# ap229997/hands

Hardware: AMD Instinct MI355X
Metric: hands/sec (higher is better)
Workload: dtype f32; 1 GPU; hands_light ResNet-50 x3 + feature_conv + HMR + MANO, 224x224, bz=256 samples/GPU (512 hands, 768 trunk passes); per_gpu_batch=256, global_batch=256, parallelism=dp1, rccl_ranks=1, launched_by=direct, conv3x3_stride1=winograd_f4x4:stages1234

## Files before the change

### hands_amd/csrc/common.h

```cpp
#pragma once
#include <hip/hip_runtime.h>
#include <math.h>

#define HANDS_LAUNCH_CHECK() return (int)hipGetLastError()

static inline int hands_grid_1d(long long work, int block, int cap = 256 * 8) {
  long long g = (work + block - 1) / block;
  if (g < 1) g = 1;
  if (g > cap) g = cap;
  return (int)g;
}

typedef float f32x4 __attribute__((ext_vector_type(4)));
typedef float f32x16 __attribute__((ext_vector_type(16)));

__device__ __forceinline__ float f4e(const float4& v, int t) {
  return t == 0 ? v.x : (t == 1 ? v.y : (t == 2 ? v.z : v.w));
}

__device__ __forceinline__ float relu_f32(float v) { return v <= 0.f ? 0.f : v; }
__device__ __forceinline__ float4 relu_f32(const float4& v) {
  return make_float4(relu_f32(v.x), relu_f32(v.y), relu_f32(v.z), relu_f32(v.w));
}
struct PoolNan4 { bool x = false, y = false, z = false, w = false; };
__device__ __forceinline__ void pool_tap(float4& m, PoolNan4& seen, const float4& v) {
  m.x = fmaxf(m.x, v.x); m.y = fmaxf(m.y, v.y); m.z = fmaxf(m.z, v.z); m.w = fmaxf(m.w, v.w);
  seen.x |= v.x != v.x; seen.y |= v.y != v.y; seen.z |= v.z != v.z; seen.w |= v.w != v.w;
}
__device__ __forceinline__ float4 pool_finish(const float4& m, const PoolNan4& seen) {
  const float q = __builtin_nanf("");
  return make_float4(seen.x ? q : m.x, seen.y ? q : m.y, seen.z ? q : m.z, seen.w ? q : m.w);
}

__device__ __forceinline__ float exp_nonpos(float x) {
  const float L2E_HI = 1.44269502162933349609375f, L2E_LO = 1.925963033500011e-08f;
// ... 61 lines not shown
```

### hands_amd/csrc/conv_igemm.hip

```cpp
#include <hip/hip_runtime.h>
#include <stdint.h>
#include "hands_hip.h"
#include "common.h"

namespace {

typedef unsigned int u32x4 __attribute__((ext_vector_type(4)));
typedef double f64x4 __attribute__((ext_vector_type(4)));

__device__ __forceinline__ float gelu_erf(float x) { return x * 0.5f * (1.0f + erff(x * 0.70710678118654752440f)); }

__device__ __forceinline__ float4 apply_act(float4 v, int act) {
  if (act == HANDS_ACT_RELU) {
    v = relu_f32(v);
  } else if (act == HANDS_ACT_GELU) {
    v.x = gelu_erf(v.x); v.y = gelu_erf(v.y); v.z = gelu_erf(v.z); v.w = gelu_erf(v.w);
  } else if (act == HANDS_ACT_LEAKY_RELU) {
    v.x = v.x > 0.f ? v.x : 0.01f * v.x; v.y = v.y > 0.f ? v.y : 0.01f * v.y;
    v.z = v.z > 0.f ? v.z : 0.01f * v.z; v.w = v.w > 0.f ? v.w : 0.01f * v.w;
  }
  return v;
}

__device__ __forceinline__ float f4elem(const float4& v, int t) {
// ... 13 lines not shown
  const float r2 = r1 - __uint_as_float(u1);
  u2 = __float_as_uint(r2);
}

__device__ __forceinline__ void store_split4(float* dst, float4 v) {
  uint32_t a0, a1, a2, b0, b1, b2, c0, c1, c2, d0, d1, d2;
  split3(v.x, a0, a1, a2); split3(v.y, b0, b1, b2); split3(v.z, c0, c1, c2); split3(v.w, d0, d1, d2);
  *reinterpret_cast<uint2*>(dst) = make_uint2((a0 >> 16) | b0, (c0 >> 16) | d0);
  *reinterpret_cast<uint2*>(dst + 8) = make_uint2((a1 >> 16) | b1, (c1 >> 16) | d1);
  *reinterpret_cast<uint2*>(dst + 16) = make_uint2((a2 >> 16) | (b2 & 0xffff0000u), (c2 >> 16) | (d2 & 0xffff0000u));
}

struct ConvArgs {
  const float* __restrict__ in;
  const float* __restrict__ w;
  const float* __restrict__ bias;
  const float* res;
  float* out;
  int M, N, Kpad;
  int H, W, Cin, Ho, Wo, KH, KW, stride, pad;
  int in_ps, out_ps, res_ps;
  int relu;
  int nblk_m, nblk_n;
  const float* __restrict__ in2;
  int K0, H2, W2, stride2, in2_ps;
  int ksplit;
  float* partial;
  int part_ps;
  const float* pre_scale;
  const float* pre_shift;
  int* counters = nullptr;
  const float* fin_res = nullptr;
  int fin_act = 0;
};

__device__ __forceinline__ int xcd_remap(int bid, int nwg) {
  const int q = nwg >> 3, r = nwg & 7;
  const int xcd = bid & 7, idx = bid >> 3;
  const int base = (xcd < r) ? xcd * (q + 1) : r * (q + 1) + (xcd - r) * q;
  return base + idx;
}

typedef float f32x2 __attribute__((ext_vector_type(2)));

constexpr int EROW = 68;
constexpr int EPI_FLOATS = 4 * 32 * EROW;
template <int ACT, bool RES>
__device__ __forceinline__ void epilogue_full(const f32x16 (&acc)[2][2], float* sE, int lane, const float* bias_p,
                                              const char* res_u, int res_ps, char* out_u, int out_ps) {
  const int half = lane >> 5;
  float* wr = sE + (lane & 31) * EROW + half * 4;
  const float* rd = sE + (lane >> 4) * EROW + (lane & 15) * 4;
  const uint32_t o_off = (uint32_t)((lane >> 4) * out_ps + (lane & 15) * 4) * 4u;
  const uint32_t r_off = (uint32_t)((lane >> 4) * res_ps + (lane & 15) * 4) * 4u;
  const float4 bv4 = *reinterpret_cast<const float4*>(bias_p);
#ifndef HANDS_EPI_SCALAR_ADDS
  const f32x2 b01 = {bv4.x, bv4.y}, b23 = {bv4.z, bv4.w};
#endif
#pragma unroll
  for (int j = 0; j < 2; ++j) {
#pragma unroll
    for (int i = 0; i < 2; ++i)
#pragma unroll
      for (int q = 0; q < 4; ++q)
        *reinterpret_cast<float4*>(wr + i * 32 + q * 8) =
            make_float4(acc[i][j][q * 4 + 0], acc[i][j][q * 4 + 1], acc[i][j][q * 4 + 2], acc[i][j][q * 4 + 3]);
    float4 rv[RES ? 8 : 1];
// ... 56 lines not shown
      float f = (float)(v + (double)a.bias[n]);
      if (a.fin_res) f += a.fin_res[(size_t)m * a.res_ps + n];
      if (a.fin_act == HANDS_ACT_RELU) f = relu_f32(f);
      else if (a.fin_act == HANDS_ACT_GELU) f = gelu_erf(f);
      else if (a.fin_act == HANDS_ACT_LEAKY_RELU) f = f > 0.f ? f : 0.01f * f;
      a.out[(size_t)m * a.out_ps + n] = f;
    }
  } else {
    constexpr int C4 = BN / 4;
    for (int idx = tid; idx < BM * C4; idx += 256) {
      const int m = m0 + idx / C4, n = n0 + (idx % C4) * 4;
      if (m >= a.M || n >= a.N) continue;
      const float* p = a.partial + (size_t)m * a.part_ps + n;
      float4 v = *reinterpret_cast<const float4*>(p);
      for (int sl = 1; sl < a.ksplit; ++sl) {
        const float4 q = *reinterpret_cast<const float4*>(p + sl * slice);
        v.x += q.x; v.y += q.y; v.z += q.z; v.w += q.w;
      }
      const float4 b = *reinterpret_cast<const float4*>(a.bias + n);
      v.x += b.x; v.y += b.y; v.z += b.z; v.w += b.w;
      if (a.fin_res) {
        const float4 r = *reinterpret_cast<const float4*>(a.fin_res + (size_t)m * a.res_ps + n);
        v.x += r.x; v.y += r.y; v.z += r.z; v.w += r.w;
      }
      *reinterpret_cast<float4*>(a.out + (size_t)m * a.out_ps + n) = apply_act(v, a.fin_act);
    }
  }
}

constexpr int SK_SLOT_FLOATS = 4 * 64 * 64;

__device__ __forceinline__ void tile_coords(const ConvArgs& a, int tile, int& mt, int& nt) {
  constexpr int RASTER_GM = 8;
  if (a.nblk_n >= 8 && a.nblk_m >= RASTER_GM) {
    const int per = RASTER_GM * a.nblk_n;
    const int gidx = tile / per, idx = tile - gidx * per;
    const int gm = min(RASTER_GM, a.nblk_m - gidx * RASTER_GM);
    nt = idx / gm; mt = gidx * RASTER_GM + (idx - nt * gm);
  } else { mt = tile / a.nblk_n; nt = tile - mt * a.nblk_n; }
}

template <int WAVES_M, int WAVES_N, int MODE, int PREC = 0, bool PRE = false, int BLK = 0>
__device__ __forceinline__ void conv_tile(const ConvArgs& a, float* lds, int tile, int split, int kt0, int kt1,
                                          const float* acc_in, float* acc_out) {
  constexpr int ROW = PREC == 1 ? LDS_ROW_B3 : LDS_ROW;
  constexpr bool F64 = PREC == 2;
  constexpr bool STEM = MODE == 1;
  constexpr bool DUAL = MODE == 2;
  constexpr int BM = 64 * WAVES_M;
  constexpr int BN = 64 * WAVES_N;
  constexpr int A_ROWS = BM / 64;
  constexpr int W_ROWS = BN / 64;
  static_assert(WAVES_M * WAVES_N == 4, "4 waves per block");

  float* sX = lds;
  float* sW = lds + 2 * BM * ROW;

  const int tid = threadIdx.x;
  const int lane = tid & 63;
  const int wave = tid >> 6;
  const int wm = wave / WAVES_N;
  const int wn = wave % WAVES_N;

  int mt, nt;
  tile_coords(a, tile, mt, nt);
  const int m0 = mt * BM, n0 = nt * BN;

  const int srow = tid >> 2;
  const int chunk = tid & 3;
  const int swz_chunk = chunk ^ ((srow >> 2) & 3);
  int x_base[A_ROWS];
  int x_hi0[A_ROWS], x_wi0[A_ROWS];
  bool x_ok[A_ROWS];
  int x_base2[DUAL ? A_ROWS : 1];
  uint32_t x_mask[MODE == 0 ? A_ROWS : 1];
  int x_offb[MODE == 0 ? A_ROWS : 1];
  int x_b[A_ROWS];
  const int HoWo = a.Ho * a.Wo;
  const bool same_pixel = DUAL && a.K0 >= a.Kpad && a.stride == 1 && a.H == a.Ho && a.W == a.Wo;
#pragma unroll
  for (int i = 0; i < A_ROWS; ++i) {
    const int m = m0 + srow + 64 * i;
    x_ok[i] = m < a.M;
    const int mm = x_ok[i] ? m : 0;
    if (same_pixel) {
      x_b[i] = 0; x_hi0[i] = 0; x_wi0[i] = 0;
      x_base[i] = mm * a.in_ps;
      if constexpr (DUAL) x_base2[i] = 0;
      continue;
    }
    const int b = mm / HoWo;
    const int rem = mm - b * HoWo;
    const int ho = rem / a.Wo;
    const int wo = rem - ho * a.Wo;
    x_b[i] = b;
    x_hi0[i] = ho * a.stride - a.pad;
    x_wi0[i] = wo * a.stride - a.pad;
    x_base[i] = ((b * a.H + x_hi0[i]) * a.W + x_wi0[i]) * a.in_ps;
    if constexpr (DUAL) {
      x_base2[i] = ((b * a.H2 + ho * a.stride2) * a.W2 + wo * a.stride2) * a.in2_ps;
    }
  }
  __amdgpu_buffer_rsrc_t x_rsrc = __builtin_amdgcn_make_buffer_rsrc(const_cast<float*>(a.in), 0, (int)0x80000000u, 0x00020000);
  if constexpr (MODE == 0) {
    const int b_w = __builtin_amdgcn_readfirstlane(x_b[0]);
    x_rsrc = __builtin_amdgcn_make_buffer_rsrc(const_cast<float*>(a.in) + (size_t)b_w * a.H * a.W * a.in_ps, 0,
                                               (int)0x80000000u, 0x00020000);
#pragma unroll
    for (int i = 0; i < A_ROWS; ++i) {
      const int hb = max(0, -x_hi0[i]), he = min(a.KH, a.H - x_hi0[i]);
      const int wb = max(0, -x_wi0[i]), we = min(a.KW, a.W - x_wi0[i]);
      const uint32_t hm = he > hb ? ((1u << he) - 1u) & ~((1u << hb) - 1u) : 0u;
      const uint32_t wm = we > wb ? ((1u << we) - 1u) & ~((1u << wb) - 1u) : 0u;
      x_mask[i] = (x_ok[i] && hm != 0u && wm != 0u) ? (hm | (wm << 16)) : 0u;
      x_offb[i] = (((((x_b[i] - b_w) * a.H + x_hi0[i]) * a.W + x_wi0[i]) * a.in_ps) + chunk * 4) * 4;
    }
  }
  int x_off1[DUAL ? A_ROWS : 1], x_off2[DUAL ? A_ROWS : 1];
  __amdgpu_buffer_rsrc_t x_rsrc2 = x_rsrc;
  if constexpr (DUAL) {
    const int base1 = __builtin_amdgcn_readfirstlane(x_base[0]);
    const int base2 = __builtin_amdgcn_readfirstlane(x_base2[0]);
    x_rsrc = __builtin_amdgcn_make_buffer_rsrc(const_cast<float*>(a.in) + base1, 0, (int)0x80000000u, 0x00020000);
    x_rsrc2 = __builtin_amdgcn_make_buffer_rsrc(const_cast<float*>(a.in2) + base2, 0, (int)0x80000000u, 0x00020000);
#pragma unroll
    for (int i = 0; i < A_ROWS; ++i) {
      x_off1[i] = x_ok[i] ? (x_base[i] - base1 + chunk * 4) * 4 : chunk * 16;
      x_off2[i] = x_ok[i] ? (x_base2[i] - base2 + chunk * 4) * 4 : chunk * 16;
    }
  }
  const __amdgpu_buffer_rsrc_t w_rsrc =
      __builtin_amdgcn_make_buffer_rsrc(const_cast<float*>(a.w) + (size_t)n0 * a.Kpad, 0, (int)0x80000000u, 0x00020000);
  int w_offb[W_ROWS];
#pragma unroll
  for (int i = 0; i < W_ROWS; ++i) w_offb[i] = ((srow + 64 * i) * a.Kpad + chunk * 4) * 4;

  float4 xr[A_ROWS], wr[W_ROWS];
  static_assert(!PRE || (MODE == 2 && PREC != 1), "the input affine + LeakyReLU exists for exact-fp32 pointwise layers");
  float4 psr = make_float4(1.f, 1.f, 1.f, 1.f), pbr = make_float4(0.f, 0.f, 0.f, 0.f);
  int kh = 0, kw = 0, c0 = 0, woff = 0;
  const int ntaps = a.KH * a.KW;
  const int cw = (a.Cin & 31) == 0 ? 2 * BK : BK;

#define LOAD_TILES(KT)                                                                              \
  do {                                                                                              \
    if constexpr (STEM) {                                                                           \
                                          \
      const int tap = (KT) * 4 + chunk;                                                             \
      const int tkh = tap / a.KW;                                                                   \
      const int tkw = tap - tkh * a.KW;                                                             \
      const int toff = (tkh * a.W + tkw) * a.in_ps;                                                 \
      _Pragma("unroll") for (int i = 0; i < A_ROWS; ++i) {                                          \
        const bool ok = x_ok[i] && tap < ntaps && (unsigned)(x_hi0[i] + tkh) < (unsigned)a.H &&     \
                        (unsigned)(x_wi0[i] + tkw) < (unsigned)a.W;                                 \
        xr[i] = ok ? *reinterpret_cast<const float4*>(a.in + (x_base[i] + toff))                    \
                   : make_float4(0.f, 0.f, 0.f, 0.f);                                               \
      }                                                                                             \
    } else if constexpr (DUAL) {                                                                    \
       \
       \
       \
      const bool second = (KT) * BK >= a.K0;                                                        \
      const int soff = ((KT) * BK - (second ? a.K0 : 0)) * 4;                                       \
      _Pragma("unroll") for (int i = 0; i < A_ROWS; ++i) {                                          \
        const u32x4 ld = second ? __builtin_amdgcn_raw_buffer_load_b128(x_rsrc2, x_off2[i], soff, 0) \
                                : __builtin_amdgcn_raw_buffer_load_b128(x_rsrc, x_off1[i], soff, 0);  \
        xr[i] = make_float4(__uint_as_float(ld.x), __uint_as_float(ld.y), __uint_as_float(ld.z), __uint_as_float(ld.w)); \
      }                                                                                             \
    } else {                                                                                        \
       \
       \
       \
      const bool kvalid = c0 < a.Cin;              \
      const uint32_t sel = kvalid ? ((1u << kh) | (0x10000u << kw)) : 0x80000000u;   \
      const int toffb = ((kh * a.W + kw) * a.in_ps + c0) * 4;                                       \
      _Pragma("unroll") for (int i = 0; i < A_ROWS; ++i) {                                          \
        const bool ok = (x_mask[i] & sel) == sel;                                                   \
        const u32x4 ld = __builtin_amdgcn_raw_buffer_load_b128(x_rsrc, ok ? x_offb[i] + toffb : (int)0x80000000u, 0, 0); \
        xr[i] = make_float4(__uint_as_float(ld.x), __uint_as_float(ld.y), __uint_as_float(ld.z), __uint_as_float(ld.w)); \
      }                                                                                             \
      woff = kvalid ? (kh * a.KW + kw) * a.Cin + c0 : (KT) * BK;                                    \
      c0 += BK;                                                                                     \
      if ((c0 & (cw - 1)) == 0) {              \
        c0 -= cw;                                                                                   \
        if (++kw == a.KW) { kw = 0; if (++kh == a.KH) { kh = 0; c0 += cw; } }                       \
      }                                                                                             \
    }                                                                                               \
    if constexpr (MODE != 0) woff = (KT) * BK;                                                      \
    if constexpr (PRE) {                                                                            \
// ... 279 lines not shown
#pragma unroll
    for (int i = 0; i < 2; ++i)
#pragma unroll
      for (int q = 0; q < 4; ++q)
        *reinterpret_cast<float4*>(sE + (lane & 31) * EROW + i * 32 + q * 8 + half * 4) =
            make_float4(acc[i][j][q * 4 + 0], acc[i][j][q * 4 + 1], acc[i][j][q * 4 + 2], acc[i][j][q * 4 + 3]);
    }
    const int mbase = m0 + wm * 64 + j * 32 + (lane >> 4);
    float4 rv[8];
#pragma unroll
    for (int r = 0; r < 8; ++r) {
      const int m = mbase + 4 * r;
      const int mc = m < a.M ? m : a.M - 1;
      rv[r] = has_res ? *reinterpret_cast<const float4*>(a.res + (size_t)mc * a.res_ps + (n_ok ? n_lane : 0))
                      : make_float4(0.f, 0.f, 0.f, 0.f);
    }
#pragma unroll
    for (int r = 0; r < 8; ++r) {
      const int m = mbase + 4 * r;
      const float4 t = *reinterpret_cast<const float4*>(sE + ((lane >> 4) + 4 * r) * EROW + c4 * 4);
      float4 v;
      v.x = t.x + bv.x + rv[r].x;
      v.y = t.y + bv.y + rv[r].y;
      v.z = t.z + bv.z + rv[r].z;
      v.w = t.w + bv.w + rv[r].w;
      v = apply_act(v, act);
      if (m < a.M && n_ok) *reinterpret_cast<float4*>(obase + (size_t)m * ops + n_lane) = v;
    }
  }
#undef LOAD_TILES
#undef STORE_TILES
}

template <int WAVES_M, int WAVES_N, int MODE, int PREC = 0, bool PRE = false, int BLK = 0>
__global__ void __launch_bounds__(256, 2) conv_igemm_f32_kernel(ConvArgs a) {
  constexpr int RING = 2 * (64 * WAVES_M + 64 * WAVES_N) * (PREC == 1 ? LDS_ROW_B3 : LDS_ROW);
  __shared__ __attribute__((aligned(16))) float lds[RING > EPI_FLOATS ? RING : EPI_FLOATS];
  const int ntiles = a.nblk_m * a.nblk_n;
  const int split = a.ksplit > 1 ? blockIdx.x / ntiles : 0;
  const int tile = xcd_remap(a.ksplit > 1 ? blockIdx.x - split * ntiles : blockIdx.x, ntiles);
  const int nk_all = a.Kpad / BK;
  const int kt0 = a.ksplit > 1 ? (int)((long long)split * nk_all / a.ksplit) : 0;
  const int kt1 = a.ksplit > 1 ? (int)((long long)(split + 1) * nk_all / a.ksplit) : nk_all;
  const int wave_u = __builtin_amdgcn_readfirstlane((int)(threadIdx.x >> 6));
  conv_tile<WAVES_M, WAVES_N, MODE, PREC, PRE, BLK>(a, lds, tile, split, kt0, kt1, nullptr, nullptr);
  if (a.ksplit > 1 && a.counters != nullptr) {
    int mt, nt;
    tile_coords(a, tile, mt, nt);
    splitk_fused_tail<64 * WAVES_M, 64 * WAVES_N, PREC == 2>(a, lds, tile, mt * 64 * WAVES_M, nt * 64 * WAVES_N, wave_u);
  }
}

constexpr int GROUP_MAX = 8;
struct GroupArgs {
  ConvArgs a[GROUP_MAX];
  int start[GROUP_MAX + 1];
  int n;
};

template <int WAVES_M, int WAVES_N, int MODE, bool PRE, int BLK>
__global__ void __launch_bounds__(256, 2) conv_igemm_group_f32_kernel(GroupArgs g) {
  constexpr int RING = 2 * (64 * WAVES_M + 64 * WAVES_N) * LDS_ROW;
  __shared__ __attribute__((aligned(16))) float lds[RING > EPI_FLOATS ? RING : EPI_FLOATS];
  int p = 0;
#pragma unroll
  for (int i = 1; i < GROUP_MAX; ++i)
    if (i < g.n && (int)blockIdx.x >= g.start[i]) p = i;
  const ConvArgs& a = g.a[p];
  const int ntiles = a.nblk_m * a.nblk_n;
  const int local = (int)blockIdx.x - g.start[p];
  if ((local >> 3) >= (ntiles >> 3) + ((local & 7) < (ntiles & 7) ? 1 : 0)) return;
  conv_tile<WAVES_M, WAVES_N, MODE, 0, PRE, BLK>(a, lds, xcd_remap(local, ntiles), 0, 0, a.Kpad / BK, nullptr, nullptr);
}

struct SkArgs {
  float* slots;
  int* flags;
  int epoch;
};

template <int WAVES_M, int WAVES_N, int MODE>
__global__ void __launch_bounds__(256, 2) conv_igemm_sk_f32_kernel(ConvArgs a, SkArgs sk) {
  constexpr int RING = 2 * (64 * WAVES_M + 64 * WAVES_N) * LDS_ROW;
  __shared__ __attribute__((aligned(16))) float lds[RING > EPI_FLOATS ? RING : EPI_FLOATS];
  __shared__ int s_ready;
  const int G = gridDim.x;
  const int g = xcd_remap(blockIdx.x, G);
  const int ntiles = a.nblk_m * a.nblk_n;
  const int nk = a.Kpad / BK;
  const long long total = (long long)ntiles * nk;
  const long long u0 = total * g / G, u1 = total * (g + 1) / G;
// ... 16 lines not shown
      tile = first_full + (sgi - head);
    } else if (inside && ka == 0) {
      tile = ta; k1 = kb;
      aout = sk.slots + (size_t)g * SK_SLOT_FLOATS;
    } else {
      if (threadIdx.x == 0) {
        int ok = 0;
        for (int spin = 0; spin < 4096 && !ok; ++spin) {
          ok = __hip_atomic_load(sk.flags + (g - 1), __ATOMIC_RELAXED, __HIP_MEMORY_SCOPE_AGENT) == sk.epoch;
          if (!ok) __builtin_amdgcn_s_sleep(8);
        }
        if (ok) __builtin_amdgcn_fence(__ATOMIC_ACQUIRE, "agent");
        s_ready = ok;
      }
      __syncthreads();
      tile = ta;
      if (s_ready != 0) { k0 = ka; ain = sk.slots + (size_t)(g - 1) * SK_SLOT_FLOATS; }
      if (inside) { k1 = kb; aout = sk.slots + (size_t)g * SK_SLOT_FLOATS; }
    }
    __syncthreads();
    conv_tile<WAVES_M, WAVES_N, MODE>(a, lds, tile, 0, k0, k1, ain, aout);
    if (aout != nullptr) {
      asm volatile("s_waitcnt vmcnt(0)" ::: "memory");
      __syncthreads();
      if (threadIdx.x == 0) {
        __builtin_amdgcn_fence(__ATOMIC_RELEASE, "agent");
        asm volatile("s_waitcnt vmcnt(0)" ::: "memory");
        if (sk.epoch > 0) __hip_atomic_store(sk.flags + g, sk.epoch, __ATOMIC_RELAXED, __HIP_MEMORY_SCOPE_AGENT);
      }
    }
  }
}

template <int WAVES_M, int WAVES_N, int MODE, int PREC = 0, bool PRE = false, int BLK = 0>
int launch(ConvArgs& a, hipStream_t stream) {
  constexpr int BM = 64 * WAVES_M, BN = 64 * WAVES_N;
  a.nblk_m = (a.M + BM - 1) / BM;
  a.nblk_n = (a.N + BN - 1) / BN;
  const long long nwg = (long long)a.nblk_m * a.nblk_n * (a.ksplit > 1 ? a.ksplit : 1);
  if (nwg <= 0 || nwg > 0x7fffffffLL) return HANDS_EINVAL;
  hipLaunchKernelGGL((conv_igemm_f32_kernel<WAVES_M, WAVES_N, MODE, PREC, PRE, BLK>), dim3((unsigned)nwg), dim3(256), 0,
                     stream, a);
  return (int)hipGetLastError();
}

template <int MODE, bool PRE = false>
int launch_fp32(const hands_conv_desc* d, ConvArgs& a, hipStream_t s) {
  const bool narrow = d->Cout <= 64;
  if (d->act & HANDS_ACC_F64) return launch<2, 2, MODE, 2, PRE>(a, s);
  if (d->act & HANDS_SUM_BLOCK128) return narrow ? launch<4, 1, MODE, 0, PRE, 8>(a, s) : launch<2, 2, MODE, 0, PRE, 8>(a, s);
  if (d->act & HANDS_SUM_BLOCK64) return narrow ? launch<4, 1, MODE, 0, PRE, 4>(a, s) : launch<2, 2, MODE, 0, PRE, 4>(a, s);
  return narrow ? launch<4, 1, MODE, 0, PRE>(a, s) : launch<2, 2, MODE, 0, PRE>(a, s);
}

constexpr int SK_MAX_G = 1024;

int device_cus() {
  static int cus = 0;
  if (cus == 0) {
    int dev = 0, n = 0;
    if (hipGetDevice(&dev) == hipSuccess &&
        hipDeviceGetAttribute(&n, hipDeviceAttributeMultiprocessorCount, dev) == hipSuccess && n > 0)
      cus = n;
    else
      cus = 256;
  }
  return cus;
}

template <int WAVES_M, int WAVES_N, int MODE>
int sk_blocks_per_cu() {
  static int occ = 0;
  if (occ == 0) {
    int n = 0;
    if (hipOccupancyMaxActiveBlocksPerMultiprocessor(&n, conv_igemm_sk_f32_kernel<WAVES_M, WAVES_N, MODE>, 256, 0) != hipSuccess || n < 1)
      n = 1;
    occ = n > 4 ? 4 : n;
  }
  return occ;
}

int streamk_grid(long long ntiles, int nk, int cus, int max_per_cu) {
  if (ntiles > cus + cus / 8 && ntiles < 2LL * cus && nk >= 128 && max_per_cu >= 2) {
    return 2 * cus;
  }
  if (nk < 16 || ntiles < 2LL * cus || ntiles > 8LL * cus) return 0;
  const double per_cu = (double)ntiles / cus;
  const long long rounds = (ntiles + cus - 1) / cus;
  if (per_cu / (double)rounds > 0.95) return 0;
  long long j = ntiles / cus;
  if (j > max_per_cu) j = max_per_cu;
  long long G = j * cus;
  if (G > SK_MAX_G) G = SK_MAX_G / cus * cus;
  return G >= cus ? (int)G : 0;
}

template <int WAVES_M, int WAVES_N, int MODE>
int launch_streamk(ConvArgs& a, hipStream_t stream, void* workspace, long long workspace_bytes, int epoch) {
  constexpr int BM = 64 * WAVES_M, BN = 64 * WAVES_N;
  a.nblk_m = (a.M + BM - 1) / BM;
  a.nblk_n = (a.N + BN - 1) / BN;
  const long long ntiles = (long long)a.nblk_m * a.nblk_n;
  const int G = (workspace && epoch != 0 && a.ksplit <= 1)
                    ? streamk_grid(ntiles, a.Kpad / BK, device_cus(), sk_blocks_per_cu<WAVES_M, WAVES_N, MODE>()) : 0;
  const long long need = (long long)G * SK_SLOT_FLOATS * 4 + (long long)SK_MAX_G * 4;
  if (G == 0 || workspace_bytes < need) return launch<WAVES_M, WAVES_N, MODE>(a, stream);
  SkArgs sk;
  sk.flags = reinterpret_cast<int*>(workspace);
  sk.slots = reinterpret_cast<float*>(reinterpret_cast<char*>(workspace) + SK_MAX_G * 4);
  sk.epoch = epoch;
  hipLaunchKernelGGL((conv_igemm_sk_f32_kernel<WAVES_M, WAVES_N, MODE>), dim3((unsigned)G), dim3(256), 0, stream, a, sk);
  return (int)hipGetLastError();
}

__global__ void splitk_reduce_kernel(const float* __restrict__ partial, int S, int M, int N4, int part_ps,
                                     const float* __restrict__ bias, const float* res, int res_ps, float* out, int out_ps,
                                     int act) {
  const long long total = (long long)M * N4;
  for (long long i = blockIdx.x * (long long)blockDim.x + threadIdx.x; i < total; i += (long long)gridDim.x * blockDim.x) {
    const int n = (int)(i % N4) * 4;
    const long long m = i / N4;
    float4 v = *reinterpret_cast<const float4*>(partial + m * part_ps + n);
    for (int s = 1; s < S; ++s) {
      const float4 p = *reinterpret_cast<const float4*>(partial + ((long long)s * M + m) * part_ps + n);
      v.x += p.x; v.y += p.y; v.z += p.z; v.w += p.w;
    }
    const float4 b = *reinterpret_cast<const float4*>(bias + n);
    v.x += b.x; v.y += b.y; v.z += b.z; v.w += b.w;
    if (res) {
      const float4 r = *reinterpret_cast<const float4*>(res + m * res_ps + n);
      v.x += r.x; v.y += r.y; v.z += r.z; v.w += r.w;
    }
    *reinterpret_cast<float4*>(out + m * out_ps + n) = apply_act(v, act);
  }
}
// ... 27 lines not shown
bool conv_geometry_ok(const hands_conv_desc* d) {
  if (d->B <= 0 || d->H <= 0 || d->W <= 0 || d->Ho <= 0 || d->Wo <= 0 || d->KH <= 0 || d->KW <= 0 || d->stride <= 0 ||
      d->pad < 0)
    return false;
  if ((d->act & HANDS_ACT_MASK) > HANDS_ACT_LEAKY_RELU || (d->act & ~(HANDS_ACT_MASK | HANDS_MATH_BF16X3 | HANDS_SUM_BLOCK128 | HANDS_SUM_BLOCK64 | HANDS_ACC_F64))) return false;
  if ((d->act & HANDS_ACC_F64) && ((d->act & (HANDS_MATH_BF16X3 | HANDS_SUM_BLOCK128 | HANDS_SUM_BLOCK64)) || d->Cin == 4)) return false;
  if ((d->act & HANDS_SUM_BLOCK128) && (d->act & (HANDS_SUM_BLOCK64 | HANDS_MATH_BF16X3))) return false;
  if ((d->act & HANDS_SUM_BLOCK64) && (d->act & HANDS_MATH_BF16X3)) return false;
  if (d->Cin % 4 || d->Cout % 4 || d->Kpad % BK || d->Kpad < d->KH * d->KW * d->Cin) return false;
  if (d->Cin != 4 && d->Cin % 16) return false;
  if (d->in_pix_stride < d->Cin || d->out_pix_stride < d->Cout) return false;
  if (d->in_pix_stride % 4 || d->out_pix_stride % 4) return false;
  if (d->H + 2 * d->pad < d->KH || d->W + 2 * d->pad < d->KW) return false;
  if (d->Ho > (d->H + 2 * d->pad - d->KH) / d->stride + 1 || d->Wo > (d->W + 2 * d->pad - d->KW) / d->stride + 1) return false;
  if ((long long)d->B * d->H * d->W * d->in_pix_stride >= (1LL << 31)) return false;
  if (d->Cin != 4) {
    const long long imgs = 256 / ((long long)d->Ho * d->Wo) + 2;
    if (imgs * d->H * d->W * d->in_pix_stride * 4 >= (1LL << 31)) return false;
    if (256LL * d->Kpad * 4 >= (1LL << 31)) return false;
    if (!(d->KH == 1 && d->KW == 1 && d->pad == 0) && (d->KH > 15 || d->KW > 15)) return false;
  }
  return true;
}

bool residual_ok(const hands_conv_desc* d, const float* residual) {
  return residual == nullptr || (d->res_pix_stride >= 0 && d->res_pix_stride % 4 == 0);
}

bool pointwise_route_ok(const hands_conv_desc* d) {
  return d->KH == 1 && d->KW == 1 && d->pad == 0 && d->Cin != 4 && d->Kpad == d->Cin &&
         (long long)(d->Ho - 1) * d->stride < d->H && (long long)(d->Wo - 1) * d->stride < d->W;
}

void fill_plain_args(const hands_conv_desc* d, const float* in, const float* w_packed, const float* bias, const float* residual,
                     float* out, const float* pre_scale, const float* pre_shift, ConvArgs& a) {
  a.in = in; a.w = w_packed; a.bias = bias; a.res = residual; a.out = out;
  a.M = d->B * d->Ho * d->Wo; a.N = d->Cout; a.Kpad = d->Kpad;
  a.H = d->H; a.W = d->W; a.Cin = d->Cin; a.Ho = d->Ho; a.Wo = d->Wo;
  a.KH = d->KH; a.KW = d->KW; a.stride = d->stride; a.pad = d->pad;
  a.in_ps = d->in_pix_stride; a.out_ps = d->out_pix_stride; a.res_ps = d->res_pix_stride;
  a.relu = d->act & HANDS_ACT_MASK;
  a.ksplit = 1; a.partial = nullptr; a.part_ps = 0; a.pre_scale = pre_scale; a.pre_shift = pre_shift;
  a.in2 = in; a.K0 = 1 << 30; a.H2 = a.W2 = a.stride2 = a.in2_ps = 0;
  a.nblk_m = a.nblk_n = 0;
}

int launch_conv(const hands_conv_desc* d, ConvArgs& a, bool pre, bool bf16x3, hipStream_t s) {
  const bool narrow = d->Cout <= 64;
  if (d->Cin == 4) return narrow ? launch<4, 1, 1>(a, s) : launch<2, 2, 1>(a, s);
  if (pre) return launch_fp32<2, true>(d, a, s);
  const bool pointwise = a.K0 < a.Kpad || pointwise_route_ok(d);
  if (bf16x3) {
    if (pointwise) return narrow ? launch<4, 1, 2, 1>(a, s) : launch<2, 2, 2, 1>(a, s);
    return narrow ? launch<4, 1, 0, 1>(a, s) : launch<2, 2, 0, 1>(a, s);
  }
  return pointwise ? launch_fp32<2>(d, a, s) : launch_fp32<0>(d, a, s);
}

int group_class(const hands_conv_desc* d, bool pre) {
  if (!d || !conv_geometry_ok(d) || !pointwise_route_ok(d)) return -1;
  if (d->act & (HANDS_MATH_BF16X3 | HANDS_SUM_BLOCK128 | HANDS_ACC_F64)) return -1;
  return (d->Cout <= 64 ? 1 : 0) | ((d->act & HANDS_SUM_BLOCK64) ? 2 : 0) | (pre ? 4 : 0);
}

template <int WAVES_M, int WAVES_N, bool PRE, int BLK>
int launch_group(GroupArgs& g, hipStream_t stream) {
  constexpr int BM = 64 * WAVES_M, BN = 64 * WAVES_N;
  long long total = 0;
  for (int p = 0; p < g.n; ++p) {
    ConvArgs& a = g.a[p];
    a.nblk_m = (a.M + BM - 1) / BM;
    a.nblk_n = (a.N + BN - 1) / BN;
    g.start[p] = (int)total;
    total += ((long long)a.nblk_m * a.nblk_n + 7) / 8 * 8;
    if (total > 0x7fffffffLL) return HANDS_EINVAL;
  }
  for (int p = g.n; p <= GROUP_MAX; ++p) g.start[p] = (int)total;
  hipLaunchKernelGGL((conv_igemm_group_f32_kernel<WAVES_M, WAVES_N, 2, PRE, BLK>), dim3((unsigned)total), dim3(256), 0, stream, g);
  return (int)hipGetLastError();
}

}

extern "C" int hands_conv2d_group_class(const hands_conv_desc* d, int pre) { return group_class(d, pre != 0); }

extern "C" int hands_conv2d_group_f32(const hands_conv_job* jobs, int n, hands_stream_t stream) {
  if (!jobs || n < 1 || n > GROUP_MAX) return HANDS_EINVAL;
  GroupArgs g{};
  g.n = n;
  int cls = -2;
  for (int p = 0; p < n; ++p) {
    const hands_conv_job& j = jobs[p];
    if (!j.desc || !j.in || !j.w_packed || !j.bias || !j.out || ((j.pre_scale != nullptr) != (j.pre_shift != nullptr))) return HANDS_EINVAL;
    const int c = group_class(j.desc, j.pre_scale != nullptr);
    if (c < 0 || (cls != -2 && c != cls)) return HANDS_EINVAL;
    if (!residual_ok(j.desc, j.residual)) return HANDS_EINVAL;
    cls = c;
    fill_plain_args(j.desc, j.in, j.w_packed, j.bias, j.residual, j.out, j.pre_scale, j.pre_shift, g.a[p]);
  }
  hipStream_t s = (hipStream_t)stream;
  switch (cls) {
    case 0: return launch_group<2, 2, false, 0>(g, s);
    case 1: return launch_group<4, 1, false, 0>(g, s);
    case 2: return launch_group<2, 2, false, 4>(g, s);
    case 3: return launch_group<4, 1, false, 4>(g, s);
    case 4: return launch_group<2, 2, true, 0>(g, s);
    case 5: return launch_group<4, 1, true, 0>(g, s);
    case 6: return launch_group<2, 2, true, 4>(g, s);
    case 7: return launch_group<4, 1, true, 4>(g, s);
  }
  return HANDS_EINVAL;
}

extern "C" int hands_conv2d_splitk_factor(const hands_conv_desc* d) { return d ? splitk_factor(d) : 0; }

extern "C" long long hands_conv2d_workspace_floats(const hands_conv_desc* d, int S) {
  if (!d || !conv_geometry_ok(d)) return -1;
  if (S <= 0) S = splitk_factor(d);
  if (S > d->Kpad / BK) S = d->Kpad / BK;
  if (S <= 1) return 0;
  return (long long)S * d->B * d->Ho * d->Wo * d->Cout * ((d->act & HANDS_ACC_F64) ? 2 : 1);
}

extern "C" int hands_conv2d_nhwc_f32(const hands_conv_desc* d, const float* in, const float* w_packed,
                                     const float* bias, const float* residual, float* out,
                                     hands_stream_t stream) {
  if (!d || !in || !w_packed || !bias || !out) return HANDS_EINVAL;
  if (!conv_geometry_ok(d) || !residual_ok(d, residual)) return HANDS_EINVAL;
  ConvArgs a;
  fill_plain_args(d, in, w_packed, bias, residual, out, nullptr, nullptr, a);
  return launch_conv(d, a, false, (d->act & HANDS_MATH_BF16X3) != 0, (hipStream_t)stream);
}

extern "C" long long hands_conv2d_streamk_workspace_bytes(void) {
  return (long long)SK_MAX_G * SK_SLOT_FLOATS * 4 + (long long)SK_MAX_G * 4;
}

extern "C" int hands_conv2d_streamk_grid(const hands_conv_desc* d) {
  if (!d || !conv_geometry_ok(d) || d->Cin == 4) return 0;
  const bool narrow = d->Cout <= 64;
  const long long M = (long long)d->B * d->Ho * d->Wo;
  const long long ntiles = narrow ? ((M + 255) / 256) * ((d->Cout + 63) / 64) : ((M + 127) / 128) * ((d->Cout + 127) / 128);
  return streamk_grid(ntiles, d->Kpad / BK, device_cus(), 4);
}

extern "C" int hands_conv2d_nhwc_streamk_f32(const hands_conv_desc* d, const float* in, const float* w_packed,
                                             const float* bias, const float* residual, float* out, void* workspace,
                                             long long workspace_bytes, int epoch, hands_stream_t stream) {
  if (!d || !in || !w_packed || !bias || !out) return HANDS_EINVAL;
  if (!conv_geometry_ok(d) || !residual_ok(d, residual)) return HANDS_EINVAL;
  if (d->Cin == 4 || (d->act & (HANDS_MATH_BF16X3 | HANDS_SUM_BLOCK128 | HANDS_SUM_BLOCK64 | HANDS_ACC_F64)))
    return hands_conv2d_nhwc_f32(d, in, w_packed, bias, residual, out, stream);
  ConvArgs a;
  fill_plain_args(d, in, w_packed, bias, residual, out, nullptr, nullptr, a);
  hipStream_t s = (hipStream_t)stream;
  if (pointwise_route_ok(d))
    return (d->Cout <= 64) ? launch_streamk<4, 1, 2>(a, s, workspace, workspace_bytes, epoch)
                           : launch_streamk<2, 2, 2>(a, s, workspace, workspace_bytes, epoch);
  return (d->Cout <= 64) ? launch_streamk<4, 1, 0>(a, s, workspace, workspace_bytes, epoch)
                         : launch_streamk<2, 2, 0>(a, s, workspace, workspace_bytes, epoch);
}

extern "C" int hands_conv1x1_dual_nhwc_f32(const hands_conv_desc* d, const float* in, const float* in2, int Cin2, int H2,
                                           int W2, int stride2, int in2_pix_stride, const float* w_packed,
                                           const float* bias, float* out, hands_stream_t stream) {
  if (!d || !in || !in2 || !w_packed || !bias || !out) return HANDS_EINVAL;
  if (d->B <= 0 || d->KH != 1 || d->KW != 1 || d->stride != 1 || d->pad != 0 || d->H != d->Ho || d->W != d->Wo)
    return HANDS_EINVAL;
  if (d->Cin % 16 || Cin2 <= 0 || Cin2 % 16 || d->Cout % 4 || d->Kpad != d->Cin + Cin2) return HANDS_EINVAL;
  if (d->in_pix_stride < d->Cin || in2_pix_stride < Cin2 || d->out_pix_stride < d->Cout || stride2 < 1) return HANDS_EINVAL;
  if (d->in_pix_stride % 4 || in2_pix_stride % 4 || d->out_pix_stride % 4) return HANDS_EINVAL;
  if ((d->Ho - 1) * stride2 >= H2 || (d->Wo - 1) * stride2 >= W2) return HANDS_EINVAL;
  if ((long long)d->B * d->H * d->W * d->in_pix_stride >= (1LL << 31) ||
      (long long)d->B * H2 * W2 * in2_pix_stride >= (1LL << 31))
    return HANDS_EINVAL;
  {
    const long long imgs = 256 / ((long long)d->Ho * d->Wo) + 2;
    if (imgs * d->H * d->W * d->in_pix_stride * 4 >= (1LL << 31) || imgs * H2 * W2 * in2_pix_stride * 4 >= (1LL << 31) ||
        256LL * d->Kpad * 4 >= (1LL << 31))
      return HANDS_EINVAL;
  }
  if (d->act & HANDS_ACC_F64) return HANDS_EINVAL;
  ConvArgs a;
  fill_plain_args(d, in, w_packed, bias, nullptr, out, nullptr, nullptr, a);
  a.in2 = in2; a.K0 = d->Cin; a.H2 = H2; a.W2 = W2; a.stride2 = stride2; a.in2_ps = in2_pix_stride;
  hands_conv_desc one_chain = *d;
  one_chain.act &= ~(HANDS_SUM_BLOCK128 | HANDS_SUM_BLOCK64);
  return launch_conv(&one_chain, a, false, (d->act & HANDS_MATH_BF16X3) != 0, (hipStream_t)stream);
}

namespace {
int splitk_launch(const hands_conv_desc* d, const float* in, const float* w_packed, const float* bias, const float* residual,
                  float* out, int S, float* workspace, long long workspace_floats,
                  hands_stream_t stream, const float* pre_scale = nullptr, const float* pre_shift = nullptr,
                  int* counters = nullptr, long long n_counters = 0) {
  if (!d) return HANDS_EINVAL;
  const bool pre = pre_scale != nullptr;
  if (pre && (!pre_shift || !pointwise_route_ok(d) || (d->act & HANDS_MATH_BF16X3))) return HANDS_EINVAL;
  const long long M = (long long)d->B * d->Ho * d->Wo;
  const int part_ps = d->Cout;
  if (S > d->Kpad / BK) S = d->Kpad / BK;
  const bool f64 = (d->act & HANDS_ACC_F64) != 0;
  const bool split = S > 1 && workspace && workspace_floats >= (long long)S * M * part_ps * (f64 ? 2 : 1) &&
                     !(f64 && (((uintptr_t)workspace) & 7));
  if (!split && !pre) return hands_conv2d_nhwc_f32(d, in, w_packed, bias, residual, out, stream);
  if (!in || !w_packed || !bias || !out || !conv_geometry_ok(d) || !residual_ok(d, residual) || (split && S > 64)) return HANDS_EINVAL;
  ConvArgs a;
  fill_plain_args(d, in, w_packed, bias, residual, out, pre_scale, pre_shift, a);
  if (split) {
    a.ksplit = S; a.partial = workspace; a.part_ps = part_ps;
    const bool narrow = d->Cout <= 64 && !f64;
    const long long ntiles = narrow ? ((M + 255) / 256) * ((d->Cout + 63) / 64) : ((M + 127) / 128) * ((d->Cout + 127) / 128);
    if (counters && n_counters >= ntiles) { a.counters = counters; a.fin_res = residual; a.fin_act = d->act & HANDS_ACT_MASK; }
  }
  hipStream_t s = (hipStream_t)stream;
  const int rc = launch_conv(d, a, pre, false, s);
  if (rc || !split || a.counters != nullptr) return rc;
  if (f64) {
    hipLaunchKernelGGL(splitk_reduce_f64_kernel, dim3(hands_grid_1d(M * d->Cout, 256)), dim3(256), 0, s,
                       reinterpret_cast<const double*>(workspace), S, (int)M, d->Cout, part_ps, bias, residual, d->res_pix_stride,
                       out, d->out_pix_stride, d->act & HANDS_ACT_MASK);
    return (int)hipGetLastError();
  }
  const long long total = M * (d->Cout / 4);
  hipLaunchKernelGGL(splitk_reduce_kernel, dim3(hands_grid_1d(total, 256)), dim3(256), 0, s, workspace, S, (int)M,
                     d->Cout / 4, part_ps, bias, residual, d->res_pix_stride, out, d->out_pix_stride, d->act & HANDS_ACT_MASK);
  return (int)hipGetLastError();
}
}

extern "C" int hands_conv2d_nhwc_pre_f32(const hands_conv_desc* d, const float* in, const float* pre_scale,
                                         const float* pre_shift, const float* w_packed, const float* bias,
                                         const float* residual, float* out, int S, float* workspace,
                                         long long workspace_floats, hands_stream_t stream) {
  if (!pre_scale || !pre_shift) return HANDS_EINVAL;
  return splitk_launch(d, in, w_packed, bias, residual, out, S, workspace, workspace_floats, stream, pre_scale, pre_shift);
}

extern "C" int hands_conv2d_nhwc_splitk_n_f32(const hands_conv_desc* d, const float* in, const float* w_packed,
                                              const float* bias, const float* residual, float* out, int S,
                                              float* workspace, long long workspace_floats, hands_stream_t stream) {
// ... 19 lines not shown
```

Baseline: 12040 hands/s.

## Add plain pointwise conv kernel and host-precomputed magic-number divisions

Replaces runtime integer divisions in tile-coordinate and pixel-index computation with host-precomputed magic multiplier/shift divisors stored in the kernel arguments. Adds a dedicated MODE 3 kernel for 1x1 stride-1 unpadded pointwise convolutions, which reads the input through buffer loads at fixed per-row offsets from a single wave-uniform base and skips per-row batch/height/width index decoding. Both the regular and stream-K launch paths route eligible pointwise convs to the new kernel. The risks are larger kernel arguments, an extra kernel instantiation, and the correctness of the magic divisor. The magic multiplier is rounded up with no add term, which is not exact for every divisor and numerator over the full 31-bit range.

Result: no change. 12010 hands/s, median of 2 (-0.2%).

```diff
diff --git a/hands_amd/csrc/common.h b/hands_amd/csrc/common.h
--- a/hands_amd/csrc/common.h
+++ b/hands_amd/csrc/common.h
@@ -1,6 +1,7 @@
 #pragma once
 #include <hip/hip_runtime.h>
 #include <math.h>
+#include "magic_div.h"
 
 #define HANDS_LAUNCH_CHECK() return (int)hipGetLastError()
 
diff --git a/hands_amd/csrc/conv_igemm.hip b/hands_amd/csrc/conv_igemm.hip
--- a/hands_amd/csrc/conv_igemm.hip
+++ b/hands_amd/csrc/conv_igemm.hip
@@ -69,7 +69,16 @@
   int* counters = nullptr;
   const float* fin_res = nullptr;
   int fin_act = 0;
+  hands_magic_div dv_howo, dv_wo, dv_nblk_n, dv_gm_tail;
 };
+
+__device__ __forceinline__ int conv_quot(const hands_magic_div& m, int n) {
+#ifdef HANDS_SETUP_DIV
+  return (int)((uint32_t)n / m.d);
+#else
+  return (int)hands_magic_quot(m, (uint32_t)n);
+#endif
+}
 
 __device__ __forceinline__ int xcd_remap(int bid, int nwg) {
   const int q = nwg >> 3, r = nwg & 7;
@@ -192,12 +201,14 @@
 
 __device__ __forceinline__ void tile_coords(const ConvArgs& a, int tile, int& mt, int& nt) {
   constexpr int RASTER_GM = 8;
+  const int row = conv_quot(a.dv_nblk_n, tile);
   if (a.nblk_n >= 8 && a.nblk_m >= RASTER_GM) {
     const int per = RASTER_GM * a.nblk_n;
-    const int gidx = tile / per, idx = tile - gidx * per;
+    const int gidx = row >> 3, idx = tile - gidx * per;
     const int gm = min(RASTER_GM, a.nblk_m - gidx * RASTER_GM);
-    nt = idx / gm; mt = gidx * RASTER_GM + (idx - nt * gm);
-  } else { mt = tile / a.nblk_n; nt = tile - mt * a.nblk_n; }
+    nt = gm == RASTER_GM ? idx >> 3 : conv_quot(a.dv_gm_tail, idx);
+    mt = gidx * RASTER_GM + (idx - nt * gm);
+  } else { mt = row; nt = tile - mt * a.nblk_n; }
 }
 
 template <int WAVES_M, int WAVES_N, int MODE, int PREC = 0, bool PRE = false, int BLK = 0>
@@ -207,6 +218,7 @@
   constexpr bool F64 = PREC == 2;
   constexpr bool STEM = MODE == 1;
   constexpr bool DUAL = MODE == 2;
+  constexpr bool PLAIN = MODE == 3;
   constexpr int BM = 64 * WAVES_M;
   constexpr int BN = 64 * WAVES_N;
   constexpr int A_ROWS = BM / 64;
@@ -219,6 +231,7 @@
   const int tid = threadIdx.x;
   const int lane = tid & 63;
   const int wave = tid >> 6;
+  const int wave_s = __builtin_amdgcn_readfirstlane(wave);
   const int wm = wave / WAVES_N;
   const int wn = wave % WAVES_N;
 
@@ -237,33 +250,30 @@
   int x_offb[MODE == 0 ? A_ROWS : 1];
   int x_b[A_ROWS];
   const int HoWo = a.Ho * a.Wo;
-  const bool same_pixel = DUAL && a.K0 >= a.Kpad && a.stride == 1 && a.H == a.Ho && a.W == a.Wo;
+  const int m_first = m0 + 16 * wave_s;
+  const int m_w = m_first < a.M ? m_first : 0;
 #pragma unroll
   for (int i = 0; i < A_ROWS; ++i) {
     const int m = m0 + srow + 64 * i;
     x_ok[i] = m < a.M;
-    const int mm = x_ok[i] ? m : 0;
-    if (same_pixel) {
-      x_b[i] = 0; x_hi0[i] = 0; x_wi0[i] = 0;
-      x_base[i] = mm * a.in_ps;
-      if constexpr (DUAL) x_base2[i] = 0;
-      continue;
-    }
-    const int b = mm / HoWo;
-    const int rem = mm - b * HoWo;
-    const int ho = rem / a.Wo;
-    const int wo = rem - ho * a.Wo;
-    x_b[i] = b;
-    x_hi0[i] = ho * a.stride - a.pad;
-    x_wi0[i] = wo * a.stride - a.pad;
-    x_base[i] = ((b * a.H + x_hi0[i]) * a.W + x_wi0[i]) * a.in_ps;
-    if constexpr (DUAL) {
-      x_base2[i] = ((b * a.H2 + ho * a.stride2) * a.W2 + wo * a.stride2) * a.in2_ps;
+    if constexpr (!PLAIN) {
+      const int mm = x_ok[i] ? m : 0;
+      const int b = conv_quot(a.dv_howo, mm);
+      const int rem = mm - b * HoWo;
+      const int ho = conv_quot(a.dv_wo, rem);
+      const int wo = rem - ho * a.Wo;
+      x_b[i] = b;
+      x_hi0[i] = ho * a.stride - a.pad;
+      x_wi0[i] = wo * a.stride - a.pad;
+      x_base[i] = ((b * a.H + x_hi0[i]) * a.W + x_wi0[i]) * a.in_ps;
+      if constexpr (DUAL) {
+        x_base2[i] = ((b * a.H2 + ho * a.stride2) * a.W2 + wo * a.stride2) * a.in2_ps;
+      }
     }
   }
   __amdgpu_buffer_rsrc_t x_rsrc = __builtin_amdgcn_make_buffer_rsrc(const_cast<float*>(a.in), 0, (int)0x80000000u, 0x00020000);
   if constexpr (MODE == 0) {
-    const int b_w = __builtin_amdgcn_readfirstlane(x_b[0]);
+    const int b_w = conv_quot(a.dv_howo, m_w);
     x_rsrc = __builtin_amdgcn_make_buffer_rsrc(const_cast<float*>(a.in) + (size_t)b_w * a.H * a.W * a.in_ps, 0,
                                                (int)0x80000000u, 0x00020000);
 #pragma unroll
@@ -276,7 +286,7 @@
       x_offb[i] = (((((x_b[i] - b_w) * a.H + x_hi0[i]) * a.W + x_wi0[i]) * a.in_ps) + chunk * 4) * 4;
     }
   }
-  int x_off1[DUAL ? A_ROWS : 1], x_off2[DUAL ? A_ROWS : 1];
+  int x_off1[(DUAL || PLAIN) ? A_ROWS : 1], x_off2[DUAL ? A_ROWS : 1];
   __amdgpu_buffer_rsrc_t x_rsrc2 = x_rsrc;
   if constexpr (DUAL) {
     const int base1 = __builtin_amdgcn_readfirstlane(x_base[0]);
@@ -288,6 +298,13 @@
       x_off1[i] = x_ok[i] ? (x_base[i] - base1 + chunk * 4) * 4 : chunk * 16;
       x_off2[i] = x_ok[i] ? (x_base2[i] - base2 + chunk * 4) * 4 : chunk * 16;
     }
+  }
+  if constexpr (PLAIN) {
+    x_rsrc = __builtin_amdgcn_make_buffer_rsrc(const_cast<float*>(a.in) + m_w * a.in_ps, 0, (int)0x80000000u, 0x00020000);
+    const int off0 = ((lane >> 2) * a.in_ps + chunk * 4) * 4;
+#pragma unroll
+    for (int i = 0; i < A_ROWS; ++i)
+      x_off1[i] = x_ok[i] ? off0 + 64 * i * a.in_ps * 4 : chunk * 16;
   }
   const __amdgpu_buffer_rsrc_t w_rsrc =
       __builtin_amdgcn_make_buffer_rsrc(const_cast<float*>(a.w) + (size_t)n0 * a.Kpad, 0, (int)0x80000000u, 0x00020000);
@@ -315,6 +332,11 @@
                         (unsigned)(x_wi0[i] + tkw) < (unsigned)a.W;                                 \
         xr[i] = ok ? *reinterpret_cast<const float4*>(a.in + (x_base[i] + toff))                    \
                    : make_float4(0.f, 0.f, 0.f, 0.f);                                               \
+      }                                                                                             \
+    } else if constexpr (PLAIN) {                                                                   \
+      _Pragma("unroll") for (int i = 0; i < A_ROWS; ++i) {                                          \
+        const u32x4 ld = __builtin_amdgcn_raw_buffer_load_b128(x_rsrc, x_off1[i], (KT) * BK * 4, 0); \
+        xr[i] = make_float4(__uint_as_float(ld.x), __uint_as_float(ld.y), __uint_as_float(ld.z), __uint_as_float(ld.w)); \
       }                                                                                             \
     } else if constexpr (DUAL) {                                                                    \
        \
@@ -660,10 +682,8 @@
 #undef STORE_TILES
 }
 
-template <int WAVES_M, int WAVES_N, int MODE, int PREC = 0, bool PRE = false, int BLK = 0>
-__global__ void __launch_bounds__(256, 2) conv_igemm_f32_kernel(ConvArgs a) {
-  constexpr int RING = 2 * (64 * WAVES_M + 64 * WAVES_N) * (PREC == 1 ? LDS_ROW_B3 : LDS_ROW);
-  __shared__ __attribute__((aligned(16))) float lds[RING > EPI_FLOATS ? RING : EPI_FLOATS];
+template <int WAVES_M, int WAVES_N, int MODE, int PREC, bool PRE, int BLK>
+__device__ __forceinline__ void conv_block(const ConvArgs& a, float* lds) {
   const int ntiles = a.nblk_m * a.nblk_n;
   const int split = a.ksplit > 1 ? blockIdx.x / ntiles : 0;
   const int tile = xcd_remap(a.ksplit > 1 ? blockIdx.x - split * ntiles : blockIdx.x, ntiles);
@@ -679,12 +699,28 @@
   }
 }
 
+template <int WAVES_M, int WAVES_N, int MODE, int PREC = 0, bool PRE = false, int BLK = 0>
+__global__ void __launch_bounds__(256, 2) conv_igemm_f32_kernel(ConvArgs a) {
+  static_assert(MODE != 3, "the plain pointwise path has a kernel of its own");
+  constexpr int RING = 2 * (64 * WAVES_M + 64 * WAVES_N) * (PREC == 1 ? LDS_ROW_B3 : LDS_ROW);
+  __shared__ __attribute__((aligned(16))) float lds[RING > EPI_FLOATS ? RING : EPI_FLOATS];
+  conv_block<WAVES_M, WAVES_N, MODE, PREC, PRE, BLK>(a, lds);
+}
+
+template <int WAVES_M, int WAVES_N>
+__global__ void __launch_bounds__(256, 2) conv_igemm_pw_f32_kernel(ConvArgs a) {
+  constexpr int RING = 2 * (64 * WAVES_M + 64 * WAVES_N) * LDS_ROW;
+  __shared__ __attribute__((aligned(16))) float lds[RING > EPI_FLOATS ? RING : EPI_FLOATS];
+  conv_block<WAVES_M, WAVES_N, 3, 0, false, 0>(a, lds);
+}
+
 constexpr int GROUP_MAX = 8;
 struct GroupArgs {
   ConvArgs a[GROUP_MAX];
   int start[GROUP_MAX + 1];
   int n;
 };
+static_assert(sizeof(GroupArgs) <= 4096, "kernel arguments: 4 KB at the most");
 
 template <int WAVES_M, int WAVES_N, int MODE, bool PRE, int BLK>
 __global__ void __launch_bounds__(256, 2) conv_igemm_group_f32_kernel(GroupArgs g) {
@@ -767,16 +803,32 @@
   }
 }
 
+template <int BM, int BN>
+bool set_tiles(ConvArgs& a) {
+  if (a.M <= 0 || a.N <= 0 || a.M > 0x7fffffff - BM) return false;
+  a.nblk_m = (a.M + BM - 1) / BM;
+  a.nblk_n = (a.N + BN - 1) / BN;
+  const int tail = a.nblk_m & 7;
+  return hands_magic_div_make(a.nblk_n, &a.dv_nblk_n) && hands_magic_div_make(tail ? tail : 8, &a.dv_gm_tail);
+}
+
 template <int WAVES_M, int WAVES_N, int MODE, int PREC = 0, bool PRE = false, int BLK = 0>
 int launch(ConvArgs& a, hipStream_t stream) {
-  constexpr int BM = 64 * WAVES_M, BN = 64 * WAVES_N;
-  a.nblk_m = (a.M + BM - 1) / BM;
-  a.nblk_n = (a.N + BN - 1) / BN;
+  if (!set_tiles<64 * WAVES_M, 64 * WAVES_N>(a)) return HANDS_EINVAL;
   const long long nwg = (long long)a.nblk_m * a.nblk_n * (a.ksplit > 1 ? a.ksplit : 1);
   if (nwg <= 0 || nwg > 0x7fffffffLL) return HANDS_EINVAL;
-  hipLaunchKernelGGL((conv_igemm_f32_kernel<WAVES_M, WAVES_N, MODE, PREC, PRE, BLK>), dim3((unsigned)nwg), dim3(256), 0,
-                     stream, a);
+  if constexpr (MODE == 3) {
+    static_assert(PREC == 0 && !PRE && BLK == 0, "the plain pointwise kernel: exact fp32, one chain");
+    hipLaunchKernelGGL((conv_igemm_pw_f32_kernel<WAVES_M, WAVES_N>), dim3((unsigned)nwg), dim3(256), 0, stream, a);
+  } else {
+    hipLaunchKernelGGL((conv_igemm_f32_kernel<WAVES_M, WAVES_N, MODE, PREC, PRE, BLK>), dim3((unsigned)nwg), dim3(256), 0,
+                       stream, a);
+  }
   return (int)hipGetLastError();
+}
+
+bool plain_pixels(const ConvArgs& a) {
+  return a.K0 >= a.Kpad && a.KH == 1 && a.KW == 1 && a.pad == 0 && a.stride == 1 && a.H == a.Ho && a.W == a.Wo;
 }
 
 template <int MODE, bool PRE = false>
@@ -785,6 +837,9 @@
   if (d->act & HANDS_ACC_F64) return launch<2, 2, MODE, 2, PRE>(a, s);
   if (d->act & HANDS_SUM_BLOCK128) return narrow ? launch<4, 1, MODE, 0, PRE, 8>(a, s) : launch<2, 2, MODE, 0, PRE, 8>(a, s);
   if (d->act & HANDS_SUM_BLOCK64) return narrow ? launch<4, 1, MODE, 0, PRE, 4>(a, s) : launch<2, 2, MODE, 0, PRE, 4>(a, s);
+  if constexpr (MODE == 2 && !PRE) {
+    if (plain_pixels(a)) return narrow ? launch<4, 1, 3>(a, s) : launch<2, 2, 3>(a, s);
+  }
   return narrow ? launch<4, 1, MODE, 0, PRE>(a, s) : launch<2, 2, MODE, 0, PRE>(a, s);
 }
 
@@ -832,10 +887,9 @@
 
 template <int WAVES_M, int WAVES_N, int MODE>
 int launch_streamk(ConvArgs& a, hipStream_t stream, void* workspace, long long workspace_bytes, int epoch) {
-  constexpr int BM = 64 * WAVES_M, BN = 64 * WAVES_N;
-  a.nblk_m = (a.M + BM - 1) / BM;
-  a.nblk_n = (a.N + BN - 1) / BN;
+  if (!set_tiles<64 * WAVES_M, 64 * WAVES_N>(a)) return HANDS_EINVAL;
   const long long ntiles = (long long)a.nblk_m * a.nblk_n;
+  if (ntiles > 0x7fffffffLL) return HANDS_EINVAL;
   const int G = (workspace && epoch != 0 && a.ksplit <= 1)
                     ? streamk_grid(ntiles, a.Kpad / BK, device_cus(), sk_blocks_per_cu<WAVES_M, WAVES_N, MODE>()) : 0;
   const long long need = (long long)G * SK_SLOT_FLOATS * 4 + (long long)SK_MAX_G * 4;
@@ -929,10 +983,15 @@
          (long long)(d->Ho - 1) * d->stride < d->H && (long long)(d->Wo - 1) * d->stride < d->W;
 }
 
-void fill_plain_args(const hands_conv_desc* d, const float* in, const float* w_packed, const float* bias, const float* residual,
+bool fill_plain_args(const hands_conv_desc* d, const float* in, const float* w_packed, const float* bias, const float* residual,
                      float* out, const float* pre_scale, const float* pre_shift, ConvArgs& a) {
+  const long long M = (long long)d->B * d->Ho * d->Wo;
+  if (M <= 0 || M > (long long)HANDS_MAGIC_MAX || !hands_magic_div_make((long long)d->Ho * d->Wo, &a.dv_howo) ||
+      !hands_magic_div_make(d->Wo, &a.dv_wo))
+    return false;
+  a.dv_nblk_n = a.dv_gm_tail = a.dv_wo;
   a.in = in; a.w = w_packed; a.bias = bias; a.res = residual; a.out = out;
-  a.M = d->B * d->Ho * d->Wo; a.N = d->Cout; a.Kpad = d->Kpad;
+  a.M = (int)M; a.N = d->Cout; a.Kpad = d->Kpad;
   a.H = d->H; a.W = d->W; a.Cin = d->Cin; a.Ho = d->Ho; a.Wo = d->Wo;
   a.KH = d->KH; a.KW = d->KW; a.stride = d->stride; a.pad = d->pad;
   a.in_ps = d->in_pix_stride; a.out_ps = d->out_pix_stride; a.res_ps = d->res_pix_stride;
@@ -940,6 +999,7 @@
   a.ksplit = 1; a.partial = nullptr; a.part_ps = 0; a.pre_scale = pre_scale; a.pre_shift = pre_shift;
   a.in2 = in; a.K0 = 1 << 30; a.H2 = a.W2 = a.stride2 = a.in2_ps = 0;
   a.nblk_m = a.nblk_n = 0;
+  return true;
 }
 
 int launch_conv(const hands_conv_desc* d, ConvArgs& a, bool pre, bool bf16x3, hipStream_t s) {
@@ -966,8 +1026,7 @@
   long long total = 0;
   for (int p = 0; p < g.n; ++p) {
     ConvArgs& a = g.a[p];
-    a.nblk_m = (a.M + BM - 1) / BM;
-    a.nblk_n = (a.N + BN - 1) / BN;
+    if (!set_tiles<BM, BN>(a)) return HANDS_EINVAL;
     g.start[p] = (int)total;
     total += ((long long)a.nblk_m * a.nblk_n + 7) / 8 * 8;
     if (total > 0x7fffffffLL) return HANDS_EINVAL;
@@ -993,7 +1052,7 @@
     if (c < 0 || (cls != -2 && c != cls)) return HANDS_EINVAL;
     if (!residual_ok(j.desc, j.residual)) return HANDS_EINVAL;
     cls = c;
-    fill_plain_args(j.desc, j.in, j.w_packed, j.bias, j.residual, j.out, j.pre_scale, j.pre_shift, g.a[p]);
+    if (!fill_plain_args(j.desc, j.in, j.w_packed, j.bias, j.residual, j.out, j.pre_scale, j.pre_shift, g.a[p])) return HANDS_EINVAL;
   }
   hipStream_t s = (hipStream_t)stream;
   switch (cls) {
@@ -1025,7 +1084,7 @@
   if (!d || !in || !w_packed || !bias || !out) return HANDS_EINVAL;
   if (!conv_geometry_ok(d) || !residual_ok(d, residual)) return HANDS_EINVAL;
   ConvArgs a;
-  fill_plain_args(d, in, w_packed, bias, residual, out, nullptr, nullptr, a);
+  if (!fill_plain_args(d, in, w_packed, bias, residual, out, nullptr, nullptr, a)) return HANDS_EINVAL;
   return launch_conv(d, a, false, (d->act & HANDS_MATH_BF16X3) != 0, (hipStream_t)stream);
 }
 
@@ -1049,8 +1108,11 @@
   if (d->Cin == 4 || (d->act & (HANDS_MATH_BF16X3 | HANDS_SUM_BLOCK128 | HANDS_SUM_BLOCK64 | HANDS_ACC_F64)))
     return hands_conv2d_nhwc_f32(d, in, w_packed, bias, residual, out, stream);
   ConvArgs a;
-  fill_plain_args(d, in, w_packed, bias, residual, out, nullptr, nullptr, a);
+  if (!fill_plain_args(d, in, w_packed, bias, residual, out, nullptr, nullptr, a)) return HANDS_EINVAL;
   hipStream_t s = (hipStream_t)stream;
+  if (pointwise_route_ok(d) && plain_pixels(a))
+    return (d->Cout <= 64) ? launch_streamk<4, 1, 3>(a, s, workspace, workspace_bytes, epoch)
+                           : launch_streamk<2, 2, 3>(a, s, workspace, workspace_bytes, epoch);
   if (pointwise_route_ok(d))
     return (d->Cout <= 64) ? launch_streamk<4, 1, 2>(a, s, workspace, workspace_bytes, epoch)
                            : launch_streamk<2, 2, 2>(a, s, workspace, workspace_bytes, epoch);
@@ -1079,7 +1141,7 @@
   }
   if (d->act & HANDS_ACC_F64) return HANDS_EINVAL;
   ConvArgs a;
-  fill_plain_args(d, in, w_packed, bias, nullptr, out, nullptr, nullptr, a);
+  if (!fill_plain_args(d, in, w_packed, bias, nullptr, out, nullptr, nullptr, a)) return HANDS_EINVAL;
   a.in2 = in2; a.K0 = d->Cin; a.H2 = H2; a.W2 = W2; a.stride2 = stride2; a.in2_ps = in2_pix_stride;
   hands_conv_desc one_chain = *d;
   one_chain.act &= ~(HANDS_SUM_BLOCK128 | HANDS_SUM_BLOCK64);
@@ -1103,7 +1165,7 @@
   if (!split && !pre) return hands_conv2d_nhwc_f32(d, in, w_packed, bias, residual, out, stream);
   if (!in || !w_packed || !bias || !out || !conv_geometry_ok(d) || !residual_ok(d, residual) || (split && S > 64)) return HANDS_EINVAL;
   ConvArgs a;
-  fill_plain_args(d, in, w_packed, bias, residual, out, pre_scale, pre_shift, a);
+  if (!fill_plain_args(d, in, w_packed, bias, residual, out, pre_scale, pre_shift, a)) return HANDS_EINVAL;
   if (split) {
     a.ksplit = S; a.partial = workspace; a.part_ps = part_ps;
     const bool narrow = d->Cout <= 64 && !f64;
diff --git a/hands_amd/csrc/magic_div.h b/hands_amd/csrc/magic_div.h
--- /dev/null
+++ b/hands_amd/csrc/magic_div.h
@@ -0,0 +1,31 @@
+#pragma once
+#include <stdint.h>
+
+#if defined(__HIPCC__)
+#define HANDS_MAGIC_HD __host__ __device__ __forceinline__
+#else
+#define HANDS_MAGIC_HD static inline
+#endif
+
+#define HANDS_MAGIC_MAX 0x7fffffffu
+
+struct hands_magic_div {
+  uint32_t mul, add, shift;
+  uint32_t d;
+};
+
+static inline bool hands_magic_div_make(long long d, hands_magic_div* m) {
+  if (d < 1 || d > (long long)HANDS_MAGIC_MAX) return false;
+  m->d = (uint32_t)d;
+  if (d == 1) { m->mul = 0xffffffffu; m->add = 0xffffffffu; m->shift = 0; return true; }
+  uint32_t s = 0;
+  while ((2ULL << s) < (unsigned long long)d) ++s;
+  m->mul = (uint32_t)(((1ULL << (32 + s)) + (unsigned long long)d - 1) / (unsigned long long)d);
+  m->add = 0;
+  m->shift = s;
+  return true;
+}
+
+HANDS_MAGIC_HD uint32_t hands_magic_quot(const hands_magic_div& m, uint32_t n) {
+  return (uint32_t)(((uint64_t)n * m.mul + m.add) >> 32) >> m.shift;
+}
```
